# GrumpyZhou/patch2pix

Hardware: AMD Instinct MI355X
Metric: image-pairs/sec (480x640, ptmax=400), matching hot path, feature pyramids resident in HBM (higher is better)
Workload: dtype f32-equivalent: fp16x2 (every f32 operand, scaled by an exact power of two, = sum of 2 fp16 planes to within 2^-24 of its magnitude; 3 fp16 MFMA products per f32 product, f32 accumulate); second convolution as Winograd F(2x2,3x3) (transforms in f32, filters transformed in f64)

## Files before the change

patch2pix_amd/csrc/consensus.hip:

```cpp
#include "coarse_common.h"

#include <algorithm>
#include <cmath>
#include <cstdlib>
#include <cstring>
#include <vector>

namespace p2p {

typedef _Float16 nh8 __attribute__((ext_vector_type(8)));
typedef float nf4 __attribute__((ext_vector_type(4)));

constexpr int NCF_THREADS = 256, NCF_WAVES = 4;
constexpr int NCF_W1_BYTES = 7 * 2 * 64 * 16;
constexpr int NCF_W2_BYTES = 5 * 2 * 64 * 16;
constexpr int NCF_C_FLOATS = 64;
constexpr int NCF_BRANCH_BYTES = NCF_W1_BYTES + NCF_W2_BYTES + NCF_C_FLOATS * 4;

struct NcFusedArgs {
    const float *X;
    float *Y;
    float *Y2;
    size_t stride;
    int d0, d1, d2, d3;
    int ta, tb, tc, td, P;
    int na, nb, nc, nd;
    const unsigned char *w;
    float b2;
    const int *xmax;
    size_t xmax_stride;
};

__host__ __device__ __forceinline__ int nc_hidden_used(int tc, int P) {
    const int n = (tc + 2) * P, r = ((n + 63) >> 6) * 64;
    return (n > r ? n : r) + 2;
}
__host__ __device__ __forceinline__ int nc_hidden_slots(int tc, int P) { return (nc_hidden_used(tc, P) + 15) & ~15; }
__host__ __device__ __forceinline__ int nc_yrow(int tc, int P) {
    int r = (tc * P + 3) & ~3;
    while ((r & 63) != 4 && (r & 63) != 12 && (r & 63) != 20 && (r & 63) != 28 && (r & 63) != 36 && (r & 63) != 44 && (r & 63) != 52 && (r & 63) != 60) r += 4;
    return r;
}
__device__ __forceinline__ int clampi(int v, int lo, int hi) { return v < lo ? lo : (v > hi ? hi : v); }
__device__ __forceinline__ unsigned short nf2h(float f) { return __builtin_bit_cast(unsigned short, (_Float16)f); }
__device__ __forceinline__ float nh2f(unsigned short b) { return (float)__builtin_bit_cast(_Float16, b); }
#define NCF_MFMA32(a, b, c) __builtin_amdgcn_mfma_f32_32x32x16_f16(__builtin_bit_cast(nh8, (a)), __builtin_bit_cast(nh8, (b)), (c), 0, 0, 0)
#define NCF_MFMA16(a, b, c) __builtin_amdgcn_mfma_f32_16x16x32_f16(__builtin_bit_cast(nh8, (a)), __builtin_bit_cast(nh8, (b)), (c), 0, 0, 0)

typedef _Float16 nh2 __attribute__((ext_vector_type(2)));
typedef float nf2 __attribute__((ext_vector_type(2)));
__device__ __forceinline__ unsigned npk(float x, float y) {
    const nf2 v = {x, y};
    return __builtin_bit_cast(unsigned, __builtin_convertvector(v, nh2));
}
__device__ __forceinline__ float npk_lo(unsigned h) { return (float)__builtin_bit_cast(nh2, h)[0]; }
__device__ __forceinline__ float npk_hi(unsigned h) { return (float)__builtin_bit_cast(nh2, h)[1]; }

#ifdef NCF_TIMING
#define NT_DECL unsigned nt_[8] = {0, 0, 0, 0, 0, 0, 0, 0}; unsigned nt_last_ = (unsigned)__builtin_amdgcn_s_memtime();
#define NT(i) { const unsigned n_ = (unsigned)__builtin_amdgcn_s_memtime(); nt_[i] += n_ - nt_last_; nt_last_ = n_; }
#else
#define NT_DECL
#define NT(i)
#endif
constexpr int NCF_KRING = 5;

template <bool FIXED>
__global__ __launch_bounds__(NCF_THREADS, 2) void nc_fused_kernel(NcFusedArgs a) {
    P2P_DYN_SHARED(unsigned char, sm);
    const int tid = threadIdx.x, lane = tid & 63, wave = __builtin_amdgcn_readfirstlane(tid >> 6);
    const int br = blockIdx.y;
    const float *X = a.X + (size_t)blockIdx.z * a.stride;
    float *Y = ((br && a.Y2) ? a.Y2 : a.Y) + (size_t)blockIdx.z * a.stride;
    const bool plain = a.Y2 != nullptr;
    int g = blockIdx.x;
    const int dt0 = (g % a.nd) * a.td; g /= a.nd;
    const int c0 = (g % a.nc) * a.tc; g /= a.nc;
    const int b0 = (g % a.nb) * a.tb; g /= a.nb;
    const int a0 = g * a.ta;
    const int TA = a.ta, TB = FIXED ? 5 : a.tb, TC = FIXED ? 8 : a.tc, TD = FIXED ? 40 : a.td, P = FIXED ? 44 : a.P;
    const int XROWS = TC + 4, HROWS = TC + 2;
    const int HNU = FIXED ? nc_hidden_used(8, 44) : nc_hidden_used(TC, P), HN = FIXED ? nc_hidden_slots(8, 44) : nc_hidden_slots(TC, P);
    const int XPLANE = (9 * XROWS * P * 2 + 8 + 15) & ~15;
    const int HKH = HN * 16, HPLANE = 2 * HKH;
    const int YROW = nc_yrow(TC, P), YSLOT = TB * YROW;
    unsigned char *Xs = sm;
    unsigned char *Hs = sm + 2 * XPLANE;
    float *Ya = (float *)(Hs + 2 * HPLANE);
    const size_t nB = (size_t)a.d2 * a.d3;

    const unsigned char *wb = a.w + (size_t)br * NCF_BRANCH_BYTES;
    nf4 w1[7][2];
#pragma unroll
    for (int s = 0; s < 7; ++s)
#pragma unroll
        for (int p = 0; p < 2; ++p) w1[s][p] = *(const nf4 *)(wb + ((s * 2 + p) * 64 + lane) * 16);
    nf4 w2[5][2];
#pragma unroll
    for (int s = 0; s < 5; ++s)
#pragma unroll
        for (int p = 0; p < 2; ++p) w2[s][p] = *(const nf4 *)(wb + NCF_W1_BYTES + ((s * 2 + p) * 64 + lane) * 16);
#pragma unroll
    for (int s = 0; s < 7; ++s)
#pragma unroll
        for (int p = 0; p < 2; ++p) P2P_OPAQUE_V4(w1[s][p]);
#pragma unroll
    for (int s = 0; s < 5; ++s)
#pragma unroll
        for (int p = 0; p < 2; ++p) P2P_OPAQUE_V4(w2[s][p]);
    const float *cf = (const float *)(wb + NCF_W1_BYTES + NCF_W2_BYTES);
    const int xeb = (a.xmax[(size_t)blockIdx.z * a.xmax_stride] >> 23) & 0xff;
    const int E = min(max(xeb - 126, 0), 100);
    const float up = __int_as_float((127 + E) << 23), down = __int_as_float((127 - E) << 23);
    const float xscale = 4096.0f * down;
    const float yun = cf[33] * up;
    float e1s[16], e1b[16];
    {
        const float hscale = cf[32] * down;
#pragma unroll
        for (int c = 0; c < 16; ++c) { e1s[c] = cf[c] * up * hscale; e1b[c] = cf[16 + c] * hscale; }
    }

    for (int i = tid; i < 3 * YSLOT; i += NCF_THREADS) Ya[i] = 0.f;
    for (int i = tid; i < 2 * HPLANE / 16; i += NCF_THREADS) *(nf4 *)(Hs + i * 16) = (nf4){0.f, 0.f, 0.f, 0.f};

    const int a_hi = min(a0 + TA, a.d0);
    const int ap_first = max(a0 - 1, 0), ap_last = min(a0 + TA, a.d0 - 1);
    const int bp_first = max(b0 - 1, 0), bp_last = min(b0 + TB, a.d1 - 1);

    auto flush = [&](int aout) {
        float *slot = Ya + (aout % 3) * YSLOT;
        const int ybase = (aout * a.d1 + b0) * (int)nB + c0 * a.d3 + dt0 + lane;
        const bool lane_in = lane < TD && dt0 + lane < a.d3;
        auto row = [&](int r) {
            const int bb = r / TC, ro = r - bb * TC;
            if (lane < TD) {
                float *cell = slot + bb * YROW + ro * P + lane + 1;
                const float v = fmaxf(*cell + a.b2, 0.f);
                *cell = 0.f;
                if (lane_in && b0 + bb < a.d1 && c0 + ro < a.d2) {
                    float *dst = Y + (unsigned)(ybase + bb * (int)nB + ro * a.d3);
                    if (plain) *dst = v; else unsafeAtomicAdd(dst, v);
                }
            }
        };
        if (FIXED) {
#pragma unroll 2
            for (int i = 0; i < 10; ++i) row(wave + NCF_WAVES * i);
        } else {
            for (int r = wave; r < TB * TC; r += NCF_WAVES) row(r);
        }
    };

    const int nbp = bp_last - bp_first + 1, nstrips = (ap_last - ap_first + 1) * nbp;
    const int sB = (int)nB, sA = a.d1 * sB;
    const int cp = min(lane & 31, P / 2 - 1), rh = lane >> 5;
    const int dcol = dt0 - 2 + 2 * cp;
    const int coff0 = clampi(dcol, 0, a.d3 - 1), coff1 = clampi(dcol + 1, 0, a.d3 - 1);
    const bool okd0 = dcol >= 0 && dcol < a.d3, okd1 = dcol + 1 >= 0 && dcol + 1 < a.d3;
    float q0v[NCF_KRING], q1v[NCF_KRING];
    int crow[NCF_KRING], lrow[NCF_KRING];
    float m0v[NCF_KRING], m1v[NCF_KRING];
#pragma unroll
    for (int k = 0; k < NCF_KRING; ++k) {
        const int it = wave + NCF_WAVES * k, i3 = min(it / 6, 2), rp = it - 6 * i3;
        const int xr = min(2 * rp + rh, XROWS - 1), ic = c0 - 2 + xr;
        crow[k] = clampi(ic, 0, a.d2 - 1) * a.d3;
        lrow[k] = (xr * P + 2 * cp) * 2;
        const bool rowok = ic >= 0 && ic < a.d2;
        m0v[k] = (rowok && okd0) ? xscale : 0.f;
        m1v[k] = (rowok && okd1) ? xscale : 0.f;
    }
    int isrc[NCF_KRING], idst[NCF_KRING];
    bool iin[NCF_KRING];
    const bool k1_second = wave >= 2;
    auto rot3 = [](int m, int i) { return m + i >= 3 ? m + i - 3 : m + i; };
    auto triple = [&](int pa, int pb, bool along_a, int ma, int mb) {
        int src3[3], dst3[3];
        bool in3[3];
#pragma unroll
        for (int i = 0; i < 3; ++i) {
            const int ia = along_a ? pa + i : pa, ib = along_a ? pb : pb + i;
            const int sa = along_a ? rot3(ma, i) : ma, sb = along_a ? mb : rot3(mb, i);
            src3[i] = clampi(ia, 0, a.d0 - 1) * sA + clampi(ib, 0, a.d1 - 1) * sB;
            in3[i] = ia >= 0 && ia < a.d0 && ib >= 0 && ib < a.d1;
            dst3[i] = (sa * 3 + sb) * XROWS * P * 2;
        }
        isrc[0] = src3[0]; iin[0] = in3[0]; idst[0] = dst3[0];
        isrc[1] = k1_second ? src3[1] : src3[0]; iin[1] = k1_second ? in3[1] : in3[0]; idst[1] = k1_second ? dst3[1] : dst3[0];
        isrc[2] = src3[1]; iin[2] = in3[1]; idst[2] = dst3[1];
        isrc[3] = src3[2]; iin[3] = in3[2]; idst[3] = dst3[2];
        isrc[4] = src3[2]; iin[4] = in3[2]; idst[4] = dst3[2];
    };
    static_assert(NCF_KRING == 5 && NCF_WAVES == 4, "the item -> plane table above");
    auto ring_load = [&]() {
#pragma unroll
        for (int k = 0; k < NCF_KRING; ++k) {
            const int src = isrc[k] + crow[k];
            q0v[k] = X[(unsigned)(src + coff0)]; q1v[k] = X[(unsigned)(src + coff1)];
        }
    };
    auto ring_store = [&]() {
#pragma unroll
        for (int k = 0; k < NCF_KRING; ++k) {
            const float f = iin[k] ? 1.f : 0.f;
            const int dst = idst[k] + lrow[k];
            const float x0 = q0v[k] * m0v[k] * f, x1 = q1v[k] * m1v[k] * f;
            const unsigned h = npk(x0, x1);
            *(unsigned *)(Xs + dst) = h;
            *(unsigned *)(Xs + XPLANE + dst) = npk(x0 - npk_lo(h), x1 - npk_hi(h));
        }
    };

    const int l31 = lane & 31, kb5 = lane >> 5;
    const int nt1 = (HROWS * P + 63) >> 6;
    int s2qh[2] = {0, 0};
    int s2dst[2] = {0, 0};
    unsigned s2ok = 0;
#pragma unroll
    for (int u = 0; u < 2; ++u) {
        const int t = wave + NCF_WAVES * u, q0 = t * 64;
        s2qh[u] = min(q0 + 2 * l31, HROWS * P - 2);
#pragma unroll
        for (int sp = 0; sp < 2; ++sp) {
            const int fl = q0 + 2 * l31 + sp, rowh = fl / P, col = fl - rowh * P;
            const int ic = c0 - 1 + rowh, id = dt0 + col - 1;
            const bool ok = t < nt1 && rowh < HROWS && col <= TD + 1 && ic >= 0 && ic < a.d2 && id >= 0 && id < a.d3;
            s2ok |= (unsigned)ok << (2 * u + sp);
        }
        s2dst[u] = (((s2ok >> (2 * u + kb5)) & 1u) ? q0 + 2 * l31 + kb5 + 1 : HNU) * 16;
    }
    const unsigned char *s2x[2] = {Xs + s2qh[0] * 2, Xs + s2qh[1] * 2};
    const int row16 = lane & 15, kb4 = lane >> 4;
    const int l2da3 = (lane & 15) / 3 % 3, l2da = (lane & 15) < 9 ? (lane & 15) / 3 : 64, l2db = (lane & 15) < 9 ? (lane & 15) % 3 : 64;
    int s3off[5];
#pragma unroll
    for (int st = 0; st < 5; ++st) {
        const int tap = min(2 * st + (kb4 >> 1), 8);
        s3off[st] = (kb4 & 1) * HKH + ((tap / 3) * P + tap % 3) * 16;
    }
    const int nt2 = (TC * P + 15) >> 4;

    auto strip_bp = [&](int ap, int j) { return (ap & 1) ? bp_last - j : bp_first + j; };
    __syncthreads();
    NT_DECL
    {
        const int bq = strip_bp(ap_first, 0);
        for (int i = 0; i < 3; ++i) {
            triple(ap_first - 1, bq - 1 + i, true, (ap_first + 2) % 3, (bq + 2 + i) % 3);
            ring_load();
            ring_store();
        }
    }
    __syncthreads();
    NT(0)
    int pending = -1;
    for (int strip = 0, row = 0, j = 0; strip < nstrips; ++strip, (j + 1 < nbp ? ++j : (j = 0, ++row))) {
        const int ap = ap_first + row, bp = strip_bp(ap, j);
        const bool more = strip + 1 < nstrips, same_row = j + 1 < nbp;
        const int dir = (ap & 1) ? -1 : 1;
        const int npa = same_row ? ap - 1 : ap + 2, npb = same_row ? bp + 2 * dir : bp - 1;
        if (pending >= 0) flush(pending);
        pending = -1;
        NT(5)
        const int am = (ap + 2) % 3, bm = (bp + 2) % 3;
        triple(npa, npb, same_row, am, same_row ? rot3(bm, dir > 0 ? 0 : 2) : bm);
        if (more) ring_load();
        {
            const int sa0 = am * 3 * XROWS * P, sa1 = rot3(am, 1) * 3 * XROWS * P, sa2 = rot3(am, 2) * 3 * XROWS * P;
            const int sl0 = bm * XROWS * P, sl1 = rot3(bm, 1) * XROWS * P, sl2 = rot3(bm, 2) * XROWS * P;
            auto xoff = [&](int gq) {
                const int da = gq / 9, db = (gq / 3) % 3, dc = gq % 3;
                return (da == 0 ? sa0 : da == 1 ? sa1 : sa2) + (db == 0 ? sl0 : db == 1 ? sl1 : sl2) + dc * P;
            };
            f32x16 acc[2] = {{0}, {0}};
            nf4 xv[2][2][2];
            auto frags = [&](int sl, nf4 (&d)[2][2]) {
                int oa0 = xoff(4 * sl), oa1 = xoff(4 * sl + 1), ob0 = xoff(4 * sl + 2), ob1 = xoff(min(4 * sl + 3, 26));
                P2P_OPAQUE_S(oa0); P2P_OPAQUE_S(oa1); P2P_OPAQUE_S(ob0); P2P_OPAQUE_S(ob1);
                const int o0 = kb5 ? ob0 : oa0, o1 = kb5 ? ob1 : oa1;
#pragma unroll
                for (int u = 0; u < 2; ++u)
#pragma unroll
                    for (int p = 0; p < 2; ++p) {
                        const unsigned *x0 = (const unsigned *)(s2x[u] + p * XPLANE + o0 * 2);
                        const unsigned *x1 = (const unsigned *)(s2x[u] + p * XPLANE + o1 * 2);
                        d[u][p] = (nf4){__uint_as_float(x0[0]), __uint_as_float(x0[1]), __uint_as_float(x1[0]), __uint_as_float(x1[1])};
                    }
            };
            frags(0, xv[0]);
#ifndef NCF_NOPRIO
            __builtin_amdgcn_s_setprio(1);
#endif
#pragma unroll
            for (int sl = 0; sl < 7; ++sl) {
                nf4 (&c)[2][2] = xv[sl & 1];
                if (sl < 6) frags(sl + 1, xv[(sl + 1) & 1]);
                acc[0] = NCF_MFMA32(w1[sl][0], c[0][1], acc[0]); acc[1] = NCF_MFMA32(w1[sl][0], c[1][1], acc[1]);
                acc[0] = NCF_MFMA32(w1[sl][1], c[0][0], acc[0]); acc[1] = NCF_MFMA32(w1[sl][1], c[1][0], acc[1]);
                acc[0] = NCF_MFMA32(w1[sl][0], c[0][0], acc[0]); acc[1] = NCF_MFMA32(w1[sl][0], c[1][0], acc[1]);
#pragma unroll
                for (int q = 0; q < 6; ++q) {
                    __builtin_amdgcn_sched_group_barrier(0x008, 1, 0);
                    __builtin_amdgcn_sched_group_barrier(0x002, 6, 0);
                    __builtin_amdgcn_sched_group_barrier(0x100, 2, 0);
                }
                __builtin_amdgcn_sched_barrier(0);
            }
            __builtin_amdgcn_s_setprio(0);
#pragma unroll
            for (int u = 0; u < 2; ++u) {
                if (wave + NCF_WAVES * u >= nt1) break;
                unsigned char *dst = Hs + s2dst[u];
#pragma unroll
                for (int kh = 0; kh < 2; ++kh) {
                    float h[8];
#pragma unroll
                    for (int j = 0; j < 4; ++j) {
                        const nf2 av = {acc[u][8 * kh + 2 * j], acc[u][8 * kh + 2 * j + 1]};
                        const nf2 sv = {e1s[8 * kh + 2 * j], e1s[8 * kh + 2 * j + 1]}, bv = {e1b[8 * kh + 2 * j], e1b[8 * kh + 2 * j + 1]};
                        const nf2 hv = __builtin_elementwise_fma(av, sv, bv);
                        h[2 * j] = fmaxf(hv[0], 0.f); h[2 * j + 1] = fmaxf(hv[1], 0.f);
                    }
                    unsigned p0[4], p1[4];
#pragma unroll
                    for (int j = 0; j < 4; ++j) {
                        p0[j] = npk(h[2 * j], h[2 * j + 1]);
                        p1[j] = npk(h[2 * j] - npk_lo(p0[j]), h[2 * j + 1] - npk_hi(p0[j]));
                    }
                    *(nf4 *)(dst + kh * HKH) = (nf4){__uint_as_float(p0[0]), __uint_as_float(p0[1]), __uint_as_float(p0[2]), __uint_as_float(p0[3])};
                    *(nf4 *)(dst + kh * HKH + HPLANE) = (nf4){__uint_as_float(p1[0]), __uint_as_float(p1[1]), __uint_as_float(p1[2]), __uint_as_float(p1[3])};
                }
            }
        }
        NT(1)
        __syncthreads();
        NT(2)
        {
            const int aout = ap + 1 - l2da, bout = bp + 1 - l2db;
            const bool lane_ok = aout >= a0 && aout < a_hi && bout >= b0 && bout < min(b0 + TB, a.d1);
            const int apm = rot3(am, 2), sl3 = apm - l2da3;
            float *ydst = Ya + (sl3 < 0 ? sl3 + 3 : sl3) * YSLOT + (bout - b0) * YROW;
            const bool yalign = (YROW & 3) == 0;
            if (FIXED) {
                const unsigned char *hl = Hs + row16 * 16;
                float *yl = ydst + 4 * kb4;
#pragma unroll
                for (int i = 0; i < 3; ++i) {
                    const int qa = (wave + 8 * i) * 16;
                    const bool has_b = i < 2 || wave < 2;
                    const int qb = has_b ? qa + 64 : qa;
                    const unsigned char *ha = hl + qa * 16, *hb = hl + qb * 16;
                    nf4 accA = {0.f, 0.f, 0.f, 0.f}, accB = {0.f, 0.f, 0.f, 0.f};
                    nf4 fr[2][4];
                    auto frags3 = [&](int st, nf4 (&d)[4]) {
                        d[0] = *(const nf4 *)(ha + s3off[st]); d[1] = *(const nf4 *)(ha + s3off[st] + HPLANE);
                        d[2] = *(const nf4 *)(hb + s3off[st]); d[3] = *(const nf4 *)(hb + s3off[st] + HPLANE);
                    };
                    frags3(0, fr[0]);
#pragma unroll
                    for (int st = 0; st < 5; ++st) {
                        nf4 (&c)[4] = fr[st & 1];
                        if (st < 4) frags3(st + 1, fr[(st + 1) & 1]);
                        __builtin_amdgcn_sched_barrier(0);
                        accA = NCF_MFMA16(c[1], w2[st][0], accA); accB = NCF_MFMA16(c[3], w2[st][0], accB);
                        accA = NCF_MFMA16(c[0], w2[st][1], accA); accB = NCF_MFMA16(c[2], w2[st][1], accB);
                        accA = NCF_MFMA16(c[0], w2[st][0], accA); accB = NCF_MFMA16(c[2], w2[st][0], accB);
                        __builtin_amdgcn_sched_barrier(0);
                    }
                    if (lane_ok) {
                        nf4 va = *(nf4 *)(yl + qa);
                        va += accA * yun;
                        *(nf4 *)(yl + qa) = va;
                        if (has_b) {
                            nf4 vb = *(nf4 *)(yl + qb);
                            vb += accB * yun;
                            *(nf4 *)(yl + qb) = vb;
                        }
                    }
                }
            } else
            for (int t = wave; t < nt2; t += 2 * NCF_WAVES) {
                const int qa = t * 16, qb = qa + NCF_WAVES * 16;
                const unsigned char *ha = Hs + min(qa + row16, TC * P - 1) * 16, *hb = Hs + min(qb + row16, TC * P - 1) * 16;
                nf4 accA = {0.f, 0.f, 0.f, 0.f}, accB = {0.f, 0.f, 0.f, 0.f};
                nf4 fr[2][4];
                auto frags3 = [&](int st, nf4 (&d)[4]) {
                    d[0] = *(const nf4 *)(ha + s3off[st]); d[1] = *(const nf4 *)(ha + s3off[st] + HPLANE);
                    d[2] = *(const nf4 *)(hb + s3off[st]); d[3] = *(const nf4 *)(hb + s3off[st] + HPLANE);
                };
                frags3(0, fr[0]);
#pragma unroll
                for (int st = 0; st < 5; ++st) {
                    nf4 (&c)[4] = fr[st & 1];
                    if (st < 4) frags3(st + 1, fr[(st + 1) & 1]);
                    __builtin_amdgcn_sched_barrier(0);
                    accA = NCF_MFMA16(c[1], w2[st][0], accA); accB = NCF_MFMA16(c[3], w2[st][0], accB);
                    accA = NCF_MFMA16(c[0], w2[st][1], accA); accB = NCF_MFMA16(c[2], w2[st][1], accB);
                    accA = NCF_MFMA16(c[0], w2[st][0], accA); accB = NCF_MFMA16(c[2], w2[st][0], accB);
                    __builtin_amdgcn_sched_barrier(0);
                }
                if (lane_ok) {
                    float *ya = ydst + qa + 4 * kb4, *yb = ydst + qb + 4 * kb4;
                    if (yalign) {
                        if (qa + 4 * kb4 + 3 < TC * P) {
                            nf4 v = *(nf4 *)ya;
                            v += accA * yun;
                            *(nf4 *)ya = v;
                        } else {
#pragma unroll
                            for (int r = 0; r < 4; ++r) if (qa + 4 * kb4 + r < TC * P) ya[r] += accA[r] * yun;
                        }
                        if (qb + 4 * kb4 + 3 < TC * P) {
                            nf4 v = *(nf4 *)yb;
                            v += accB * yun;
                            *(nf4 *)yb = v;
                        } else {
#pragma unroll
                            for (int r = 0; r < 4; ++r) if (qb + 4 * kb4 + r < TC * P) yb[r] += accB[r] * yun;
                        }
                    } else {
#pragma unroll
                        for (int r = 0; r < 4; ++r) {
                            if (qa + 4 * kb4 + r < TC * P) ya[r] += accA[r] * yun;
                            if (qb + 4 * kb4 + r < TC * P) yb[r] += accB[r] * yun;
                        }
                    }
                }
            }
        }
        NT(3)
        if (more) ring_store();
        NT(4)
        if (!same_row && ap - 1 >= a0) pending = ap - 1;
        __syncthreads();
        NT(6)
    }
    if (pending >= 0) flush(pending);
    if (nstrips > 0 && ap_last < a_hi && ap_last >= a0) flush(ap_last);
#ifdef NCF_TIMING
    if (blockIdx.x == 5 && blockIdx.y == 0 && lane == 0) {
        __syncthreads();
        for (int i = 0; i < 8; ++i) Y[wave * 8 + i] = (float)nt_[i];
        Y[32] = (float)nstrips;
    }
#endif
}

static void put2(unsigned char *frag, int lane, int j, float v) {
    uint16_t *d = (uint16_t *)frag;
    split_fp16_planes(v, &d[lane * 8 + j], &d[(64 + lane) * 8 + j]);
}

void pack_nc_fused(const float *w1, const float *b1, const float *w2, DeviceBlob &out) {
    unsigned char *const bytes = out.at<unsigned char>(out.take<unsigned char>(2 * NCF_BRANCH_BYTES));
    auto W1 = [&](int o, int da, int db, int dc, int dd) { return w1[(((da * 16 + o) * 3 + db) * 3 + dc) * 3 + dd]; };
    auto W2 = [&](int c, int da, int db, int dc, int dd) { return w2[(((da * 16 + c) * 3 + db) * 3 + dc) * 3 + dd]; };
    for (int br = 0; br < 2; ++br) {
        auto W1b = [&](int o, int da, int db, int dc, int dd) { return br ? W1(o, dc, dd, da, db) : W1(o, da, db, dc, dd); };
        auto W2b = [&](int c, int da, int db, int dc, int dd) { return br ? W2(c, dc, dd, da, db) : W2(c, da, db, dc, dd); };
        unsigned char *base = bytes + (size_t)br * NCF_BRANCH_BYTES;
        int t1[16];
        float hmax = 0.f, w2max = 0.f;
        for (int o = 0; o < 16; ++o) {
            float mx = 0.f, sum = std::fabs(b1[o]);
            for (int t = 0; t < 81; ++t) {
                const float v = W1b(o, t / 27, (t / 9) % 3, (t / 3) % 3, t % 3);
                mx = std::max(mx, std::fabs(v));
                sum += std::fabs(v);
            }
            t1[o] = pow2_exponent_to(mx, 12);
            hmax = std::max(hmax, sum);
            for (int t = 0; t < 81; ++t) w2max = std::max(w2max, std::fabs(W2b(o, t / 27, (t / 9) % 3, (t / 3) % 3, t % 3)));
        }
        const int sh = pow2_exponent_to(2.f * hmax, 13), t2 = pow2_exponent_to(w2max, 12);
        for (int sl = 0; sl < 7; ++sl)
            for (int lane = 0; lane < 64; ++lane)
                for (int j = 0; j < 8; ++j) {
                    const int k = sl * 16 + 8 * (lane >> 5) + j, gq = k >> 2, e = k & 3;
                    const int n = lane & 31, s = (n >> 2) & 1, o = (n & 3) + 4 * (n >> 3), dd = e - s;
                    float v = 0.f;
                    if (gq < 27 && dd >= 0 && dd <= 2) v = std::ldexp(W1b(o, gq / 9, (gq / 3) % 3, gq % 3, dd), t1[o]);
                    put2(base + sl * 2 * 64 * 16, lane, j, v);
                }
        for (int st = 0; st < 5; ++st)
            for (int lane = 0; lane < 64; ++lane)
                for (int j = 0; j < 8; ++j) {
                    const int kb = lane >> 4, tap = 2 * st + (kb >> 1), ch = 8 * (kb & 1) + j, n = lane & 15;
                    float v = 0.f;
                    if (tap < 9 && n < 9) v = std::ldexp(W2b(ch, n / 3, n % 3, tap / 3, tap % 3), t2);
                    put2(base + NCF_W1_BYTES + st * 2 * 64 * 16, lane, j, v);
                }
        float *cf = (float *)(base + NCF_W1_BYTES + NCF_W2_BYTES);
        for (int o = 0; o < 16; ++o) {
            cf[o] = std::ldexp(1.f, -12 - t1[o]);
            cf[16 + o] = b1[o];
        }
        cf[32] = std::ldexp(1.f, sh);
        cf[33] = std::ldexp(1.f, -sh - t2);
    }
}

size_t nc_fused_lds_bytes(int tb, int tc, int P) {
    return (size_t)2 * ((9 * (tc + 4) * P * 2 + 8 + 15) & ~15) + (size_t)2 * 2 * nc_hidden_slots(tc, P) * 16 + (size_t)3 * tb * nc_yrow(tc, P) * 4 + 256;
}

__global__ __launch_bounds__(256) void absmax_kernel(const float *__restrict__ x, size_t n, size_t stride, int *out, size_t out_stride) {
    __shared__ float part[4];
    x += (size_t)blockIdx.z * stride;
    float m = 0.f;
    const size_t n4 = (((size_t)x & 15) == 0) ? n >> 2 : 0;
    const size_t step = (size_t)gridDim.x * 256;
    size_t i = (size_t)blockIdx.x * 256 + threadIdx.x;
    for (; i + 3 * step < n4; i += 4 * step) {
        const nf4 v0 = ((const nf4 *)x)[i], v1 = ((const nf4 *)x)[i + step], v2 = ((const nf4 *)x)[i + 2 * step], v3 = ((const nf4 *)x)[i + 3 * step];
        m = fmaxf(fmaxf(m, fmaxf(fabsf(v0[0]), fabsf(v0[1]))), fmaxf(fabsf(v0[2]), fabsf(v0[3])));
        m = fmaxf(fmaxf(m, fmaxf(fabsf(v1[0]), fabsf(v1[1]))), fmaxf(fabsf(v1[2]), fabsf(v1[3])));
        m = fmaxf(fmaxf(m, fmaxf(fabsf(v2[0]), fabsf(v2[1]))), fmaxf(fabsf(v2[2]), fabsf(v2[3])));
        m = fmaxf(fmaxf(m, fmaxf(fabsf(v3[0]), fabsf(v3[1]))), fmaxf(fabsf(v3[2]), fabsf(v3[3])));
    }
    for (; i < n4; i += step) {
        const nf4 v = ((const nf4 *)x)[i];
        m = fmaxf(fmaxf(m, fmaxf(fabsf(v[0]), fabsf(v[1]))), fmaxf(fabsf(v[2]), fabsf(v[3])));
    }
    for (size_t j = 4 * n4 + (size_t)blockIdx.x * 256 + threadIdx.x; j < n; j += step) m = fmaxf(m, fabsf(x[j]));
#pragma unroll
    for (int d = 32; d >= 1; d >>= 1) m = fmaxf(m, __shfl_xor(m, d));
    if ((threadIdx.x & 63) == 0) part[threadIdx.x >> 6] = m;
    __syncthreads();
    if (threadIdx.x == 0) {
        const float mm = fmaxf(fmaxf(part[0], part[1]), fmaxf(part[2], part[3]));
        int *dst = out + (size_t)blockIdx.z * out_stride;
        if (__float_as_int(mm) > *(volatile int *)dst) atomicMax(dst, __float_as_int(mm));
    }
}

int launch_absmax(const float *x, size_t n, size_t stride, int pairs, int *out, size_t out_stride, hipStream_t stream) {
    const unsigned blocks = (unsigned)std::min<size_t>((n + 16383) / 16384, 256);
    hipLaunchKernelGGL(absmax_kernel, dim3(blocks, 1, pairs), dim3(256), 0, stream, x, n, stride, out, out_stride);
    return check_launch("absmax_kernel");
}

static long nc_fused_tile(NcFusedArgs &a, int pairs, const int *forced) {
    const int d0 = a.d0, d1 = a.d1, d2 = a.d2, d3 = a.d3;
    a.nd = ceil_div(d3, 60);
    a.td = ceil_div(d3, a.nd);
    a.P = (a.td + 4 + 1) & ~1;
    a.tb = 5; a.tc = 8; a.ta = 0;
    if (forced && forced[1] > 0 && forced[2] > 0) { a.ta = forced[0]; a.tb = forced[1]; a.tc = forced[2]; }
    a.tb = std::min(a.tb, d1); a.tc = std::min(a.tc, d2);
    while (a.tc > 1 && (a.tc + 4 > 12 || (a.tc + 2) * a.P > 512)) --a.tc;
    a.nb = ceil_div(d1, a.tb); a.nc = ceil_div(d2, a.tc);
    if (a.ta <= 0) {
        a.ta = d0;
        while (a.ta > 4 && (long)ceil_div(d0, a.ta) * a.nb * a.nc * a.nd * 2 * pairs < 1024) a.ta = (a.ta + 1) / 2;
    }
    a.ta = std::min(a.ta, d0);
    a.na = ceil_div(d0, a.ta);
    return (long)a.na * a.nb * a.nc * a.nd * 2 * pairs;
}

int launch_nc_fused(const float *X, float *Y, float *Y2, size_t stride, int pairs, int d0, int d1, int d2, int d3,
                    const unsigned char *w_dev, float b2, const int *xmax, size_t xmax_stride, const int *forced_tile,
                    hipStream_t stream) {
    P2P_REQUIRE((unsigned long long)d0 * d1 * d2 * d3 < (1ull << 31), P2P_EUNSUPPORTED,
                "consensus volume %d x %d x %d x %d has 2^31 cells or more", d0, d1, d2, d3);
    NcFusedArgs a{};
    a.X = X; a.Y = Y; a.Y2 = Y2; a.stride = stride; a.d0 = d0; a.d1 = d1; a.d2 = d2; a.d3 = d3; a.w = w_dev; a.b2 = b2;
    a.xmax = xmax; a.xmax_stride = xmax_stride;
    nc_fused_tile(a, pairs, forced_tile);
    const size_t lds = nc_fused_lds_bytes(a.tb, a.tc, a.P);
    P2P_REQUIRE(a.P <= 64 && lds <= 160 * 1024 && a.tc + 4 <= 12 && (a.tc + 2) * a.P <= 512, P2P_EUNSUPPORTED,
                "consensus tile does not fit (P %d, tc %d, LDS %zu)", a.P, a.tc, lds);
    static DeviceOnce attr_set;
    const int dev = raise_lds_limit(attr_set, {{(const void *)nc_fused_kernel<false>, 160 * 1024}, {(const void *)nc_fused_kernel<true>, 160 * 1024}});
    if (dev < 0) return dev;
    if (a.tb == 5 && a.tc == 8 && a.td == 40 && a.P == 44)
        hipLaunchKernelGGL(nc_fused_kernel<true>, dim3(a.na * a.nb * a.nc * a.nd, 2, pairs), dim3(NCF_THREADS), lds, stream, a);
    else
        hipLaunchKernelGGL(nc_fused_kernel<false>, dim3(a.na * a.nb * a.nc * a.nd, 2, pairs), dim3(NCF_THREADS), lds, stream, a);
    return check_launch("nc_fused_kernel");
}

}
```

Measured before the change: 926.2.

## Run both consensus branches in one 512-thread block sharing the staged input tile

The two branches of the fused consensus kernel now run together in a single 512-thread block, four waves per branch, instead of one block per branch. The staged fp16 input planes in LDS are loaded once and shared, which halves global input traffic and staging work per tile. Each branch keeps its own hidden and output buffers. The tiler now weighs tb=10 against tb=5 using an occupancy slot count and halo cost, and adds a tb=10 specialisation. The trade-off is one block per CU at higher LDS use, fewer concurrent blocks, and a reworked ring-load table.

```diff
diff --git a/patch2pix_amd/csrc/consensus.hip b/patch2pix_amd/csrc/consensus.hip
--- a/patch2pix_amd/csrc/consensus.hip
+++ b/patch2pix_amd/csrc/consensus.hip
@@ -11,7 +11,7 @@
 typedef _Float16 nh8 __attribute__((ext_vector_type(8)));
 typedef float nf4 __attribute__((ext_vector_type(4)));
 
-constexpr int NCF_THREADS = 256, NCF_WAVES = 4;
+constexpr int NCF_THREADS = 512, NCF_WAVES = 8, NCF_HWAVES = 4;
 constexpr int NCF_W1_BYTES = 7 * 2 * 64 * 16;
 constexpr int NCF_W2_BYTES = 5 * 2 * 64 * 16;
 constexpr int NCF_C_FLOATS = 64;
@@ -63,13 +63,16 @@
 #define NT_DECL
 #define NT(i)
 #endif
-constexpr int NCF_KRING = 5;
-
-template <bool FIXED>
-__global__ __launch_bounds__(NCF_THREADS, 2) void nc_fused_kernel(NcFusedArgs a) {
+constexpr int NCF_KRING = 3;
+
+__host__ __device__ __forceinline__ int nc_xplane(int tc, int P) { return (9 * (tc + 4) * P * 2 + 15) & ~15; }
+
+template <int FTB>
+__global__ __launch_bounds__(NCF_THREADS, 1) void nc_fused_kernel(NcFusedArgs a) {
     P2P_DYN_SHARED(unsigned char, sm);
+    constexpr bool FIXED = FTB > 0;
     const int tid = threadIdx.x, lane = tid & 63, wave = __builtin_amdgcn_readfirstlane(tid >> 6);
-    const int br = blockIdx.y;
+    const int br = wave >> 2, hw = wave & 3;
     const float *X = a.X + (size_t)blockIdx.z * a.stride;
     float *Y = ((br && a.Y2) ? a.Y2 : a.Y) + (size_t)blockIdx.z * a.stride;
     const bool plain = a.Y2 != nullptr;
@@ -78,15 +81,15 @@
     const int c0 = (g % a.nc) * a.tc; g /= a.nc;
     const int b0 = (g % a.nb) * a.tb; g /= a.nb;
     const int a0 = g * a.ta;
-    const int TA = a.ta, TB = FIXED ? 5 : a.tb, TC = FIXED ? 8 : a.tc, TD = FIXED ? 40 : a.td, P = FIXED ? 44 : a.P;
+    const int TA = a.ta, TB = FIXED ? FTB : a.tb, TC = FIXED ? 8 : a.tc, TD = FIXED ? 40 : a.td, P = FIXED ? 44 : a.P;
     const int XROWS = TC + 4, HROWS = TC + 2;
     const int HNU = FIXED ? nc_hidden_used(8, 44) : nc_hidden_used(TC, P), HN = FIXED ? nc_hidden_slots(8, 44) : nc_hidden_slots(TC, P);
-    const int XPLANE = (9 * XROWS * P * 2 + 8 + 15) & ~15;
+    const int XPLANE = FIXED ? nc_xplane(8, 44) : nc_xplane(TC, P);
     const int HKH = HN * 16, HPLANE = 2 * HKH;
     const int YROW = nc_yrow(TC, P), YSLOT = TB * YROW;
     unsigned char *Xs = sm;
-    unsigned char *Hs = sm + 2 * XPLANE;
-    float *Ya = (float *)(Hs + 2 * HPLANE);
+    unsigned char *Hs = sm + 2 * XPLANE + br * 2 * HPLANE;
+    float *Ya = (float *)(sm + 2 * XPLANE + 4 * HPLANE) + br * 3 * YSLOT;
     const size_t nB = (size_t)a.d2 * a.d3;
 
     const unsigned char *wb = a.w + (size_t)br * NCF_BRANCH_BYTES;
@@ -121,8 +124,8 @@
         for (int c = 0; c < 16; ++c) { e1s[c] = cf[c] * up * hscale; e1b[c] = cf[16 + c] * hscale; }
     }
 
-    for (int i = tid; i < 3 * YSLOT; i += NCF_THREADS) Ya[i] = 0.f;
-    for (int i = tid; i < 2 * HPLANE / 16; i += NCF_THREADS) *(nf4 *)(Hs + i * 16) = (nf4){0.f, 0.f, 0.f, 0.f};
+    for (int i = tid; i < 2 * 3 * YSLOT; i += NCF_THREADS) ((float *)(sm + 2 * XPLANE + 4 * HPLANE))[i] = 0.f;
+    for (int i = tid; i < 4 * HPLANE / 16; i += NCF_THREADS) *(nf4 *)(sm + 2 * XPLANE + i * 16) = (nf4){0.f, 0.f, 0.f, 0.f};
 
     const int a_hi = min(a0 + TA, a.d0);
     const int ap_first = max(a0 - 1, 0), ap_last = min(a0 + TA, a.d0 - 1);
@@ -146,9 +149,9 @@
         };
         if (FIXED) {
 #pragma unroll 2
-            for (int i = 0; i < 10; ++i) row(wave + NCF_WAVES * i);
+            for (int i = 0; i < 2 * FTB; ++i) row(hw + NCF_HWAVES * i);
         } else {
-            for (int r = wave; r < TB * TC; r += NCF_WAVES) row(r);
+            for (int r = hw; r < TB * TC; r += NCF_HWAVES) row(r);
         }
     };
 
@@ -173,7 +176,7 @@
     }
     int isrc[NCF_KRING], idst[NCF_KRING];
     bool iin[NCF_KRING];
-    const bool k1_second = wave >= 2;
+    const bool k0_second = wave >= 6, k1_third = wave >= 4;
     auto rot3 = [](int m, int i) { return m + i >= 3 ? m + i - 3 : m + i; };
     auto triple = [&](int pa, int pb, bool along_a, int ma, int mb) {
         int src3[3], dst3[3];
@@ -186,13 +189,11 @@
             in3[i] = ia >= 0 && ia < a.d0 && ib >= 0 && ib < a.d1;
             dst3[i] = (sa * 3 + sb) * XROWS * P * 2;
         }
-        isrc[0] = src3[0]; iin[0] = in3[0]; idst[0] = dst3[0];
-        isrc[1] = k1_second ? src3[1] : src3[0]; iin[1] = k1_second ? in3[1] : in3[0]; idst[1] = k1_second ? dst3[1] : dst3[0];
-        isrc[2] = src3[1]; iin[2] = in3[1]; idst[2] = dst3[1];
-        isrc[3] = src3[2]; iin[3] = in3[2]; idst[3] = dst3[2];
-        isrc[4] = src3[2]; iin[4] = in3[2]; idst[4] = dst3[2];
+        isrc[0] = k0_second ? src3[1] : src3[0]; iin[0] = k0_second ? in3[1] : in3[0]; idst[0] = k0_second ? dst3[1] : dst3[0];
+        isrc[1] = k1_third ? src3[2] : src3[1]; iin[1] = k1_third ? in3[2] : in3[1]; idst[1] = k1_third ? dst3[2] : dst3[1];
+        isrc[2] = src3[2]; iin[2] = in3[2]; idst[2] = dst3[2];
     };
-    static_assert(NCF_KRING == 5 && NCF_WAVES == 4, "the item -> plane table above");
+    static_assert(NCF_KRING == 3 && NCF_WAVES == 8, "the item -> plane table above");
     auto ring_load = [&]() {
 #pragma unroll
         for (int k = 0; k < NCF_KRING; ++k) {
@@ -219,7 +220,7 @@
     unsigned s2ok = 0;
 #pragma unroll
     for (int u = 0; u < 2; ++u) {
-        const int t = wave + NCF_WAVES * u, q0 = t * 64;
+        const int t = hw + NCF_HWAVES * u, q0 = t * 64;
         s2qh[u] = min(q0 + 2 * l31, HROWS * P - 2);
 #pragma unroll
         for (int sp = 0; sp < 2; ++sp) {
@@ -310,7 +311,7 @@
             __builtin_amdgcn_s_setprio(0);
 #pragma unroll
             for (int u = 0; u < 2; ++u) {
-                if (wave + NCF_WAVES * u >= nt1) break;
+                if (hw + NCF_HWAVES * u >= nt1) break;
                 unsigned char *dst = Hs + s2dst[u];
 #pragma unroll
                 for (int kh = 0; kh < 2; ++kh) {
@@ -347,8 +348,8 @@
                 float *yl = ydst + 4 * kb4;
 #pragma unroll
                 for (int i = 0; i < 3; ++i) {
-                    const int qa = (wave + 8 * i) * 16;
-                    const bool has_b = i < 2 || wave < 2;
+                    const int qa = (hw + 8 * i) * 16;
+                    const bool has_b = i < 2 || hw < 2;
                     const int qb = has_b ? qa + 64 : qa;
                     const unsigned char *ha = hl + qa * 16, *hb = hl + qb * 16;
                     nf4 accA = {0.f, 0.f, 0.f, 0.f}, accB = {0.f, 0.f, 0.f, 0.f};
@@ -380,8 +381,8 @@
                     }
                 }
             } else
-            for (int t = wave; t < nt2; t += 2 * NCF_WAVES) {
-                const int qa = t * 16, qb = qa + NCF_WAVES * 16;
+            for (int t = hw; t < nt2; t += 2 * NCF_HWAVES) {
+                const int qa = t * 16, qb = qa + NCF_HWAVES * 16;
                 const unsigned char *ha = Hs + min(qa + row16, TC * P - 1) * 16, *hb = Hs + min(qb + row16, TC * P - 1) * 16;
                 nf4 accA = {0.f, 0.f, 0.f, 0.f}, accB = {0.f, 0.f, 0.f, 0.f};
                 nf4 fr[2][4];
@@ -439,9 +440,9 @@
     if (pending >= 0) flush(pending);
     if (nstrips > 0 && ap_last < a_hi && ap_last >= a0) flush(ap_last);
 #ifdef NCF_TIMING
-    if (blockIdx.x == 5 && blockIdx.y == 0 && lane == 0) {
-        __syncthreads();
-        for (int i = 0; i < 8; ++i) Y[wave * 8 + i] = (float)nt_[i];
+    __syncthreads();
+    if (blockIdx.x == 5 && br == 0 && lane == 0) {
+        for (int i = 0; i < 8; ++i) Y[hw * 8 + i] = (float)nt_[i];
         Y[32] = (float)nstrips;
     }
 #endif
@@ -502,7 +503,7 @@
 }
 
 size_t nc_fused_lds_bytes(int tb, int tc, int P) {
-    return (size_t)2 * ((9 * (tc + 4) * P * 2 + 8 + 15) & ~15) + (size_t)2 * 2 * nc_hidden_slots(tc, P) * 16 + (size_t)3 * tb * nc_yrow(tc, P) * 4 + 256;
+    return (size_t)2 * nc_xplane(tc, P) + 2 * ((size_t)2 * 2 * nc_hidden_slots(tc, P) * 16 + (size_t)3 * tb * nc_yrow(tc, P) * 4);
 }
 
 __global__ __launch_bounds__(256) void absmax_kernel(const float *__restrict__ x, size_t n, size_t stride, int *out, size_t out_stride) {
@@ -541,23 +542,39 @@
     return check_launch("absmax_kernel");
 }
 
+constexpr size_t NCF_LDS_MAX = 160 * 1024;
+constexpr int NCF_SLOTS = 256;
+
 static long nc_fused_tile(NcFusedArgs &a, int pairs, const int *forced) {
     const int d0 = a.d0, d1 = a.d1, d2 = a.d2, d3 = a.d3;
     a.nd = ceil_div(d3, 60);
     a.td = ceil_div(d3, a.nd);
     a.P = (a.td + 4 + 1) & ~1;
-    a.tb = 5; a.tc = 8; a.ta = 0;
-    if (forced && forced[1] > 0 && forced[2] > 0) { a.ta = forced[0]; a.tb = forced[1]; a.tc = forced[2]; }
-    a.tb = std::min(a.tb, d1); a.tc = std::min(a.tc, d2);
+    a.tc = 8;
+    const bool forced_bc = forced && forced[1] > 0 && forced[2] > 0;
+    if (forced_bc) a.tc = forced[2];
+    a.tc = std::min(a.tc, d2);
     while (a.tc > 1 && (a.tc + 4 > 12 || (a.tc + 2) * a.P > 512)) --a.tc;
-    a.nb = ceil_div(d1, a.tb); a.nc = ceil_div(d2, a.tc);
-    if (a.ta <= 0) {
-        a.ta = d0;
-        while (a.ta > 4 && (long)ceil_div(d0, a.ta) * a.nb * a.nc * a.nd * 2 * pairs < 1024) a.ta = (a.ta + 1) / 2;
-    }
-    a.ta = std::min(a.ta, d0);
-    a.na = ceil_div(d0, a.ta);
-    return (long)a.na * a.nb * a.nc * a.nd * 2 * pairs;
+    a.nc = ceil_div(d2, a.tc);
+    const int forced_ta = forced_bc ? forced[0] : 0;
+    long best = -1;
+    int best_ta = 0, best_tb = 0;
+    for (int cand : {10, 5}) {
+        int tb = std::min(forced_bc ? forced[1] : cand, d1);
+        while (tb > 1 && nc_fused_lds_bytes(tb, a.tc, a.P) > NCF_LDS_MAX) --tb;
+        const long per_a = (long)ceil_div(d1, tb) * a.nc * a.nd * pairs;
+        int ta = forced_ta > 0 ? forced_ta : d0;
+        if (forced_ta <= 0)
+            while (ta > 4 && ceil_div(d0, ta) * per_a < NCF_SLOTS) ta = (ta + 1) / 2;
+        ta = std::min(ta, d0);
+        const long groups = ceil_div(d0, ta) * per_a;
+        const long cost = (groups + NCF_SLOTS - 1) / NCF_SLOTS * (ta + 2) * (tb + 2);
+        if (best < 0 || cost < best) { best = cost; best_ta = ta; best_tb = tb; }
+        if (forced_bc) break;
+    }
+    a.ta = best_ta; a.tb = best_tb;
+    a.na = ceil_div(d0, a.ta); a.nb = ceil_div(d1, a.tb);
+    return (long)a.na * a.nb * a.nc * a.nd * pairs;
 }
 
 int launch_nc_fused(const float *X, float *Y, float *Y2, size_t stride, int pairs, int d0, int d1, int d2, int d3,
@@ -570,15 +587,20 @@
     a.xmax = xmax; a.xmax_stride = xmax_stride;
     nc_fused_tile(a, pairs, forced_tile);
     const size_t lds = nc_fused_lds_bytes(a.tb, a.tc, a.P);
-    P2P_REQUIRE(a.P <= 64 && lds <= 160 * 1024 && a.tc + 4 <= 12 && (a.tc + 2) * a.P <= 512, P2P_EUNSUPPORTED,
+    P2P_REQUIRE(a.P <= 64 && lds <= NCF_LDS_MAX && a.tc + 4 <= 12 && (a.tc + 2) * a.P <= 512, P2P_EUNSUPPORTED,
                 "consensus tile does not fit (P %d, tc %d, LDS %zu)", a.P, a.tc, lds);
     static DeviceOnce attr_set;
-    const int dev = raise_lds_limit(attr_set, {{(const void *)nc_fused_kernel<false>, 160 * 1024}, {(const void *)nc_fused_kernel<true>, 160 * 1024}});
+    const int dev = raise_lds_limit(attr_set, {{(const void *)nc_fused_kernel<0>, (int)NCF_LDS_MAX}, {(const void *)nc_fused_kernel<5>, (int)NCF_LDS_MAX},
+                                               {(const void *)nc_fused_kernel<10>, (int)NCF_LDS_MAX}});
     if (dev < 0) return dev;
-    if (a.tb == 5 && a.tc == 8 && a.td == 40 && a.P == 44)
-        hipLaunchKernelGGL(nc_fused_kernel<true>, dim3(a.na * a.nb * a.nc * a.nd, 2, pairs), dim3(NCF_THREADS), lds, stream, a);
+    const dim3 grid(a.na * a.nb * a.nc * a.nd, 1, pairs);
+    const bool fixed = a.tc == 8 && a.td == 40 && a.P == 44;
+    if (fixed && a.tb == 10)
+        hipLaunchKernelGGL(nc_fused_kernel<10>, grid, dim3(NCF_THREADS), lds, stream, a);
+    else if (fixed && a.tb == 5)
+        hipLaunchKernelGGL(nc_fused_kernel<5>, grid, dim3(NCF_THREADS), lds, stream, a);
     else
-        hipLaunchKernelGGL(nc_fused_kernel<false>, dim3(a.na * a.nb * a.nc * a.nd, 2, pairs), dim3(NCF_THREADS), lds, stream, a);
+        hipLaunchKernelGGL(nc_fused_kernel<0>, grid, dim3(NCF_THREADS), lds, stream, a);
     return check_launch("nc_fused_kernel");
 }
 
```

Result: faster. 938.9, median of 6 (+1.4%).
